# caskcsg/lightretriever

Measured on AMD Instinct MI355X. Metric: docs embedded/sec (llama3.2-1b dims, seq_len=512, bf16) [+ queries/sec@top-100 over 1000000-doc index in `search`], higher is better.
Workload: dtype bf16

## Files before the change

### lightretriever_amd/csrc/lrx_common.h

```cpp
#pragma once
#include <hip/hip_runtime.h>
#include <stdint.h>
#include <stdio.h>
#include <string.h>
#include "../../include/lrx.h"

typedef __attribute__((ext_vector_type(8))) __bf16 bf16x8;
typedef __attribute__((ext_vector_type(4))) __bf16 bf16x4;
typedef __attribute__((ext_vector_type(2))) __bf16 bf16x2;
typedef __attribute__((ext_vector_type(4))) short s16x4;
typedef __attribute__((ext_vector_type(2))) float f32x2;
typedef __attribute__((ext_vector_type(4))) float f32x4;
typedef __attribute__((ext_vector_type(16))) float f32x16;
typedef __attribute__((ext_vector_type(4))) uint32_t u32x4;
typedef __attribute__((ext_vector_type(2))) uint32_t u32x2;

#define LRX_WAVE 64

__device__ __forceinline__ float bf2f(__bf16 v) { return (float)v; }
__device__ __forceinline__ __bf16 f2bf(float v) { return (__bf16)v; }
__device__ __forceinline__ float bfbits2f(uint32_t lo16) { return __uint_as_float(lo16 << 16); }

__device__ __forceinline__ float wave_sum(float v) {
#pragma unroll
// ... 15 lines not shown
}
__device__ __forceinline__ float key2f(uint32_t k) {
  uint32_t u = (k & 0x80000000u) ? (k & 0x7FFFFFFFu) : ~k;
  return __uint_as_float(u);
}
__device__ __forceinline__ unsigned long long sel_pack(uint32_t key, int64_t i) {
  return ((unsigned long long)key << 32) | (unsigned long long)(0xFFFFFFFFu - (uint32_t)i);
}
__device__ __forceinline__ int64_t sel_row(unsigned long long c) { return (int64_t)(0xFFFFFFFFu - (uint32_t)(c & 0xFFFFFFFFull)); }

__host__ __device__ __forceinline__ int64_t lrx_shadow_off(int64_t r, int k, int D) {
  return ((r >> 7) * (int64_t)(D / 64) + (k >> 6)) * 8192 + ((((r >> 4) & 7) * 2 + ((k >> 5) & 1)) * 64 + ((k >> 3) & 3) * 16 + (r & 15)) * 8 + (k & 7);
}

#ifdef LRX_DEV_KNOBS
#include <stdlib.h>
static inline int lrx_dev_knob(const char* name, int dflt) { const char* e = getenv(name); return e ? atoi(e) : dflt; }
#else
static inline int lrx_dev_knob(const char*, int dflt) { return dflt; }
#endif

void lrx_set_error(const char* fmt, ...);
#define LRX_CHECK_ARG(cond, ...)          \
  do {                                    \
    if (!(cond)) {                        \
      lrx_set_error(__VA_ARGS__);         \
      return LRX_ERR_INVALID;             \
    }                                     \
  } while (0)
#define LRX_HIP(call)                                                                     \
  do {                                                                                    \
    hipError_t e_ = (call);                                                               \
    if (e_ != hipSuccess) {                                                               \
      lrx_set_error("%s failed: %s (%s:%d)", #call, hipGetErrorString(e_), __FILE__, __LINE__); \
      return LRX_ERR_HIP;                                                                 \
    }                                                                                     \
  } while (0)
#define LRX_LAUNCH_CHECK() LRX_HIP(hipGetLastError())

static inline int64_t lrx_cdiv(int64_t a, int64_t b) { return (a + b - 1) / b; }

#define LRX_EMIT_MAX_QUERIES 1024
int lrx_gemm_filter_emit_launch(const void* Xb, const void* q16, int64_t n_rows, int nq, int dim, int ss, int64_t n_tiles,
                                const float* thr, unsigned long long* cand, unsigned int* cnt, unsigned int cap, hipStream_t stream);
int lrx_gemm_filter_sample_launch(const void* Xb, const void* q16, int64_t n_rows, int nq, int dim, int ss, int64_t n_tiles, float* scores, float* gmax,
                                  int64_t ld_s, int nblk_ld_s, hipStream_t stream);
int lrx_gemm_max_aggregate_launch(const void* A, const void* B, const void* bias, const int32_t* row_seg, float* out, int64_t ldo, int M, int N,
                                  int K, hipStream_t stream);

int lrx_gemm_nt_fused_ex(const void* A, const void* B, void* C, const void* bias, const void* resid, int32_t M, int32_t N, int32_t K, int32_t epilogue,
                         const float* rscale, float* ss_part, int f16, void* stream);
int lrx_gemm_qkv_rope_slice_ex(const void* A, const void* Wqkv, void* C, const void* bias, const int32_t* positions, const float* cos, const float* sin,
                               int32_t M, int32_t K, int32_t num_q_heads, int32_t num_kv_heads, int32_t head_dim, const float* rscale, int32_t head0,
                               int32_t n_heads, int f16, void* stream);
int lrx_gemm_nt_resid32_ex(const void* A, const void* B, float* x32, void* a16_out, const void* gamma, int32_t M, int32_t N, int32_t K, float* ss_part,
                           int f16, int out_f16, void* stream);
int lrx_attn_varlen_causal_ex(const void* qkv, const int32_t* cu_seqlens, const void* items, size_t items_bytes, int32_t n_seqs, int32_t total_tokens,
                              int32_t max_seqlen, int32_t num_q_heads, int32_t num_kv_heads, int32_t head_dim, void* out, int32_t last_tile_only,
                              int out_f16, void* stream);
int lrx_attn_prefix_suffix_ex(const void* qkv, const void* prefix_kv, int32_t n_seqs, int32_t suffix_len, int32_t prefix_len, int32_t num_q_heads,
                              int32_t num_kv_heads, int32_t head_dim, void* out, int out_f16, void* stream);
int lrx_embed_stream32_ex(const void* table, const int32_t* ids, int32_t n_tokens, int32_t hidden, int32_t vocab, const void* gamma, float* x32, void* a16,
                          float* rscale, float eps, int f16, void* stream);
int lrx_pool_sum_rows(const void* src, int src_kind, const int32_t* ids, int vocab, const int32_t* cu_seqlens, int n_seqs, int hidden_size, float* aux,
                      hipStream_t stream);
int lrx_pool_norm_aux(const void* hidden, const void* final_norm_w, const int32_t* cu_seqlens, int32_t n_seqs, int32_t hidden_size, float eps,
                      int32_t pooling, const float* aux, float* out, int64_t out_row_stride, int32_t out_dim, int32_t normalize, void* shadow_out,
                      int64_t shadow_row0, float* row_bounds, int32_t hidden_f32, void* stream);
int lrx_gather_rows_u32(const void* src, const int32_t* cu_seqlens, int32_t n_seqs, void* dst, hipStream_t stream);
```

### lightretriever_amd/csrc/lrx_gemm.hip

```cpp
#include "lrx_common.h"
#include <float.h>
#include <stdlib.h>

#define GBM 256
#define GBN 256
#define GBK 64
#define HALF_BYTES 16384

enum { EPI_STORE = 0, EPI_RESID = 1, EPI_SWIGLU = 2, EPI_ROPE = 3, EPI_MAXAGG = 4, EPI_EMIT = 5, EPI_RESID32 = 6, EPI_SAMPLE = 7 };
#define EPI_IS_SEARCH(E) ((E) == EPI_EMIT || (E) == EPI_SAMPLE)

struct RopeArgs {
  const int32_t* positions;
  const float* cos;
  const float* sin;
  int rope_cols;
  int head_dim;
  int ldc;
};

__device__ __forceinline__ __bf16 f2h_bits(float v) {
  return __builtin_bit_cast(__bf16, (_Float16)fminf(fmaxf(v, -65504.f), 65504.f));
}
__device__ unsigned int g_qkv_fp16_saturations = 0;
// ... 16 lines not shown
  float* scores;
  float* gmax;
  int64_t ld_s;
  int nblk_ld_s;
};

struct MaxAggArgs {
  const int32_t* row_seg;
  float* out;
  int64_t ldo;
};

struct NormArgs {
  const float* rscale;
  float* ss_part;
  int group_m;
};

__device__ __forceinline__ void atomic_fmax_bits(float* p, float v) {
  const unsigned b = __float_as_uint(v);
  if (!(b & 0x80000000u)) __hip_atomic_fetch_max((int*)p, (int)b, __ATOMIC_RELAXED, __HIP_MEMORY_SCOPE_AGENT);
  else __hip_atomic_fetch_min((unsigned*)p, b, __ATOMIC_RELAXED, __HIP_MEMORY_SCOPE_AGENT);
}

typedef const __attribute__((address_space(1))) void* gptr_t;
typedef __attribute__((address_space(3))) void* lptr_t;

#define G_BAR()                            \
  do {                                     \
    __builtin_amdgcn_sched_barrier(0);     \
    __builtin_amdgcn_s_barrier();          \
    __builtin_amdgcn_sched_barrier(0);     \
  } while (0)
#define G_LSYNC()                                          \
  do {                                                     \
    asm volatile("s_waitcnt lgkmcnt(0)" ::: "memory");     \
    G_BAR();                                               \
  } while (0)



typedef __attribute__((ext_vector_type(8))) _Float16 f16x8;
template <int EPI, bool F16>
__device__ __forceinline__ f32x4 gemm_mfma(bf16x8 x, bf16x8 y, f32x4 c) {
  if constexpr (EPI_IS_SEARCH(EPI) || F16) return __builtin_amdgcn_mfma_f32_16x16x32_f16(__builtin_bit_cast(f16x8, x), __builtin_bit_cast(f16x8, y), c, 0, 0, 0);
  else return __builtin_amdgcn_mfma_f32_16x16x32_bf16(x, y, c, 0, 0, 0);
}

template <int EPI, bool F16 = false, bool OUTH = F16>
__global__ void __launch_bounds__(512, 2)
k_gemm_bf16_nt(const __bf16* __restrict__ A, const __bf16* __restrict__ B, __bf16* C, const __bf16* __restrict__ bias,
               const __bf16* resid, int M, int N, int K, int tiles_m, int tiles_n, RopeArgs rope, MaxAggArgs mx, NormArgs nrm, EmitArgs em) {
  __shared__ __attribute__((aligned(1024))) char smem[8 * HALF_BYTES + (EPI == EPI_EMIT ? 2304 : 0)];
  const int nwg = gridDim.x, bid = blockIdx.x;
  const int xcd = bid & 7, qd = nwg >> 3, rm = nwg & 7;
  const int t_lin = (xcd < rm ? xcd * (qd + 1) : rm * (qd + 1) + (xcd - rm) * qd) + (bid >> 3);
  const int GM = nrm.group_m;
  const int width = GM * tiles_n;
  const int group = t_lin / width, first_m = group * GM;
  const int gsz = min(tiles_m - first_m, GM);
  const int tin = t_lin - group * width;
  const int tm = first_m + tin % gsz, tn = tin / gsz;
  const int tmx = EPI == EPI_SAMPLE ? tm * em.ss : ((EPI == EPI_EMIT && em.ss > 1) ? (tm / (em.ss - 1)) * em.ss + 1 + tm % (em.ss - 1) : tm);
  const int m0 = tmx * GBM, n0 = tn * GBN;

  const int tid = threadIdx.x, lane = tid & 63;
  const int wave = __builtin_amdgcn_readfirstlane(tid >> 6);
  const int wr = wave >> 2, wc = wave & 3;
  if constexpr (EPI == EPI_EMIT) {
    float* xthr = (float*)(smem + 8 * HALF_BYTES);
    unsigned int* xqc = (unsigned int*)(smem + 8 * HALF_BYTES + 1024);
    if (tid < GBN) { xthr[tid] = n0 + tid < N ? em.thr[n0 + tid] : FLT_MAX; xqc[tid] = 0u; }
    if (tid < 8) ((unsigned int*)(smem + 8 * HALF_BYTES + 2048))[tid] = 0u;
  }

  const __bf16 *pA0[2], *pA1[2], *pB0[2], *pB1[2];
#pragma unroll
  for (int i = 0; i < 2; ++i) {
    int s = (wave * 2 + i) * 64 + lane;
    int row = s >> 3, c = (s & 7) ^ ((row >> 1) & 7);
    if (EPI_IS_SEARCH(EPI)) {
      const int64_t lastb = (int64_t)(M - 1) >> 7;
      const int64_t b0 = min((int64_t)(m0 >> 7), lastb), b1 = min((int64_t)(m0 >> 7) + 1, lastb);
      pA0[i] = A + (b0 * (K / 64)) * 8192 + s * 8;
      pA1[i] = A + (b1 * (K / 64)) * 8192 + s * 8;
    } else {
      pA0[i] = A + (int64_t)min(m0 + row, M - 1) * K + c * 8;
      pA1[i] = A + (int64_t)min(m0 + 128 + row, M - 1) * K + c * 8;
    }
    pB0[i] = B + (int64_t)min(n0 + row, N - 1) * K + c * 8;
    pB1[i] = B + (int64_t)min(n0 + 128 + row, N - 1) * K + c * 8;
  }
  char* const dma_dst = smem + wave * 2048;
#define G_KOFF(KT) ((KT) * GBK)
  const int a_ks = EPI_IS_SEARCH(EPI) ? 8192 : GBK;
#define G_ISSUE_(P, SLOT, BUF, KOFF)                                                                                       \
  do {                                                                                                                     \
    __builtin_amdgcn_global_load_lds((gptr_t)(P[0] + (KOFF)), (lptr_t)(dma_dst + (BUF) * 65536 + (SLOT) * HALF_BYTES), 16, 0, 0);        \
    __builtin_amdgcn_global_load_lds((gptr_t)(P[1] + (KOFF)), (lptr_t)(dma_dst + (BUF) * 65536 + (SLOT) * HALF_BYTES + 1024), 16, 0, 0); \
  } while (0)
#define G_ISSUE(P, SLOT, BUF, KT) G_ISSUE_(P, SLOT, BUF, ((SLOT) < 2 ? (int64_t)(KT) * a_ks : (int64_t)G_KOFF(KT)))

  const int fr = lane & 15, fq = lane >> 4;
  const int xs = fr >> 1;
  int laneoff[2];
#pragma unroll
  for (int ks = 0; ks < 2; ++ks) laneoff[ks] = fr * 128 + (((ks * 4 + fq) ^ xs) << 4);
  int laneoffA[2];
#pragma unroll
  for (int ks = 0; ks < 2; ++ks) laneoffA[ks] = EPI_IS_SEARCH(EPI) ? ks * 1024 + lane * 16 : laneoff[ks];
  const int a_off = (wr * 64) * 128, b_off = 2 * HALF_BYTES + (wc * 32) * 128;

  f32x4 acc[2][2][4][2];
#pragma unroll
  for (int h = 0; h < 2; ++h)
#pragma unroll
    for (int hp = 0; hp < 2; ++hp)
#pragma unroll
      for (int mi = 0; mi < 4; ++mi)
#pragma unroll
        for (int ni = 0; ni < 2; ++ni) acc[h][hp][mi][ni] = f32x4{0.f, 0.f, 0.f, 0.f};
  bf16x8 a[4][2], b[2][2];

#define G_LDA(H)                                                                                     \
  _Pragma("unroll") for (int mi = 0; mi < 4; ++mi) _Pragma("unroll") for (int ks = 0; ks < 2; ++ks)  \
      a[mi][ks] = *(const bf16x8*)(sbuf + (H) * HALF_BYTES + a_off + mi * 2048 + laneoffA[ks]);
#define G_LDB(HP)                                                                                    \
  _Pragma("unroll") for (int ni = 0; ni < 2; ++ni) _Pragma("unroll") for (int ks = 0; ks < 2; ++ks)  \
      b[ni][ks] = *(const bf16x8*)(sbuf + (HP) * HALF_BYTES + b_off + ni * 2048 + laneoff[ks]);
#define G_MM(H, HP)                                                                                   \
  do {                                                                                                \
    _Pragma("unroll") for (int ks = 0; ks < 2; ++ks) _Pragma("unroll") for (int mi = 0; mi < 4; ++mi) \
        _Pragma("unroll") for (int ni = 0; ni < 2; ++ni) acc[H][HP][mi][ni] =                        \
            gemm_mfma<EPI, F16>(b[ni][ks], a[mi][ks], acc[H][HP][mi][ni]); \
  } while (0)

  float rsv[2][4];
#pragma unroll
  for (int h = 0; h < 2; ++h)
#pragma unroll
    for (int mi = 0; mi < 4; ++mi)
      rsv[h][mi] = (EPI != EPI_MAXAGG && EPI != EPI_RESID && !EPI_IS_SEARCH(EPI) && nrm.rscale != nullptr) ? nrm.rscale[min(m0 + h * 128 + wr * 64 + mi * 16 + fr, M - 1)] : 1.0f;

  int rposv[2][4];
#pragma unroll
  for (int h = 0; h < 2; ++h)
#pragma unroll
    for (int mi = 0; mi < 4; ++mi) rposv[h][mi] = EPI == EPI_ROPE ? rope.positions[min(m0 + h * 128 + wr * 64 + mi * 16 + fr, M - 1)] : 0;

  const int nk = K / GBK;
  G_ISSUE(pA0, 0, 0, 0); G_ISSUE(pB1, 3, 0, 0); G_ISSUE(pA1, 1, 0, 0); G_ISSUE(pB0, 2, 0, 0);
  if (nk > 1) {
    G_ISSUE(pA0, 0, 1, 1); G_ISSUE(pB0, 2, 1, 1); G_ISSUE(pB1, 3, 1, 1); G_ISSUE(pA1, 1, 1, 1);
    asm volatile("s_waitcnt vmcnt(8)" ::: "memory");
  } else {
    asm volatile("s_waitcnt vmcnt(0)" ::: "memory");
  }

  G_BAR();
  if (wr == 1) G_BAR();

  bf16x8 b2[2][2];
#define G_LDB2(HP)                                                                                   \
  _Pragma("unroll") for (int ni = 0; ni < 2; ++ni) _Pragma("unroll") for (int ks = 0; ks < 2; ++ks)  \
      b2[ni][ks] = *(const bf16x8*)(sbuf + (HP) * HALF_BYTES + b_off + ni * 2048 + laneoff[ks]);
#define G_MM2(H, HP)                                                                                  \
  do {                                                                                                \
    _Pragma("unroll") for (int ks = 0; ks < 2; ++ks) _Pragma("unroll") for (int mi = 0; mi < 4; ++mi) \
        _Pragma("unroll") for (int ni = 0; ni < 2; ++ni) acc[H][HP][mi][ni] =                        \
            gemm_mfma<EPI, F16>(b2[ni][ks], a[mi][ks], acc[H][HP][mi][ni]); \
  } while (0)
  for (int t = 0; t < nk; ++t) {
    const int cur = t & 1;
    const char* sbuf = smem + cur * 65536;
    const bool n1 = t + 1 < nk, n2 = t + 2 < nk;
    G_LDB(0) G_LDB2(1) G_LDA(0)
    if (t >= 1 && n1) G_ISSUE(pA1, 1, cur ^ 1, t + 1);
    if (n1 && n2) asm volatile("s_waitcnt vmcnt(8)" ::: "memory"); else asm volatile("s_waitcnt vmcnt(0)" ::: "memory");
    G_LSYNC();
    __builtin_amdgcn_s_setprio(1);
    G_MM(0, 0); G_MM2(0, 1);
    __builtin_amdgcn_s_setprio(0);
    G_BAR();
    G_LDA(1)
    if (n2) {
      G_ISSUE(pA0, 0, cur, t + 2); G_ISSUE(pB0, 2, cur, t + 2); G_ISSUE(pB1, 3, cur, t + 2);
      asm volatile("s_waitcnt vmcnt(8)" ::: "memory");
    } else {
      asm volatile("s_waitcnt vmcnt(0)" ::: "memory");
    }
    G_LSYNC();
    __builtin_amdgcn_s_setprio(1);
    G_MM2(1, 1); G_MM(1, 0);
    __builtin_amdgcn_s_setprio(0);
    G_BAR();
  }
  if (wr == 0) G_BAR();

  if constexpr (EPI == EPI_SAMPLE) {
    const int64_t gstride = 8 * (int64_t)em.nblk_ld_s;
#pragma unroll
    for (int hp = 0; hp < 2; ++hp) {
      if (hp) __syncthreads();
#pragma unroll
      for (int h = 0; h < 2; ++h)
#pragma unroll
        for (int mi = 0; mi < 4; ++mi) {
          const int row = h * 128 + wr * 64 + mi * 16 + fr;
          const bool mok = (int64_t)m0 + row < M;
#pragma unroll
          for (int ni = 0; ni < 2; ++ni)
#pragma unroll
            for (int r = 0; r < 4; ++r) {
              const int cl = wc * 32 + ni * 16 + fq * 4 + r;
              *(float*)(smem + cl * 1024 + ((((row >> 2) ^ (fq << 2))) << 4) + (row & 3) * 4) = mok ? acc[h][hp][mi][ni][r] : -FLT_MAX;
            }
        }
      __syncthreads();
#pragma unroll 4
      for (int it = 0; it < 16; ++it) {
        const int cl = it * 8 + wave, col = n0 + hp * 128 + cl;
        const f32x4 v = *(const f32x4*)(smem + cl * 1024 + ((lane ^ (((cl >> 2) & 3) << 2)) << 4));
        float mx = fmaxf(fmaxf(v[0], v[1]), fmaxf(v[2], v[3]));
        mx = fmaxf(mx, __int_as_float(__builtin_amdgcn_update_dpp(0, __float_as_int(mx), 0x4E, 0xF, 0xF, true)));
        mx = fmaxf(mx, __int_as_float(__builtin_amdgcn_update_dpp(0, __float_as_int(mx), 0xB1, 0xF, 0xF, true)));
        if (col < N) {
          *(f32x4*)(em.scores + (int64_t)col * em.ld_s + (int64_t)tm * GBM + lane * 4) = v;
          if ((lane & 3) == 0) em.gmax[(int64_t)col * gstride + (int64_t)tm * 16 + (lane >> 2)] = mx;
        }
      }
    }
    return;
  }
  if constexpr (EPI == EPI_EMIT) {
    constexpr int WCAP = 512;
    unsigned long long* wl = (unsigned long long*)(smem + wave * (WCAP * 12 + 64));
    unsigned int* wq = (unsigned int*)(wl + WCAP);
    unsigned int* wn = (unsigned int*)(smem + 8 * HALF_BYTES + 2048) + wave;
    unsigned int* qc = (unsigned int*)(smem + 8 * HALF_BYTES + 1024);
    const float* xthr = (const float*)(smem + 8 * HALF_BYTES);
    f32x4 t16[2][2];
#pragma unroll
    for (int hp = 0; hp < 2; ++hp)
#pragma unroll
      for (int ni = 0; ni < 2; ++ni) t16[hp][ni] = *(const f32x4*)(xthr + hp * 128 + wc * 32 + ni * 16 + fq * 4);
#pragma unroll
    for (int h = 0; h < 2; ++h)
#pragma unroll
      for (int mi = 0; mi < 4; ++mi) {
        const int64_t m = (int64_t)m0 + h * 128 + wr * 64 + mi * 16 + fr;
// ... 54 lines not shown
#pragma unroll
      for (int it = 0; it < 16; ++it) {
        const int m = m0 + p * 128 + it * 8 + wave;
        rv[it] = (m < M && nin) ? *(const f32x4*)(x32 + (int64_t)m * N + nq4) : f32x4{0.f, 0.f, 0.f, 0.f};
      }
      if (p) __syncthreads();
#pragma unroll
      for (int hp = 0; hp < 2; ++hp)
#pragma unroll
        for (int mi = 0; mi < 4; ++mi)
#pragma unroll
          for (int ni = 0; ni < 2; ++ni) {
            const int row = wr * 64 + mi * 16 + fr, chunk = hp * 32 + wc * 8 + ni * 4 + fq;
            *(f32x4*)(smem + row * 1024 + ((chunk ^ ((row & 15) << 2)) << 4)) = acc[p][hp][mi][ni];
          }
      __syncthreads();
#pragma unroll
      for (int it = 0; it < 16; ++it) {
        const int row = it * 8 + wave, m = m0 + p * 128 + row;
        f32x4 v = *(const f32x4*)(smem + row * 1024 + ((lane ^ ((row & 15) << 2)) << 4));
        const bool inb = m < M && nin;
#pragma unroll
        for (int e = 0; e < 4; ++e) v[e] += rv[it][e];
        if (inb) {
          *(f32x4*)(x32 + (int64_t)m * N + nq4) = v;
          if (C != nullptr) {
            bf16x4 a4;
            if constexpr (OUTH) {
              bool sat = false;
#pragma unroll
              for (int e = 0; e < 4; ++e) { const float t = v[e] * gm[e]; sat |= !(fabsf(t) <= 65504.f); a4[e] = f2h_bits(t); }
              if (__any(sat)) { if ((int)(threadIdx.x & 63) == __ffsll((long long)__ballot(1)) - 1) atomicAdd(&g_qkv_fp16_saturations, 1u); }
            } else {
#pragma unroll
              for (int e = 0; e < 4; ++e) a4[e] = f2bf(v[e] * gm[e]);
            }
            *(bf16x4*)(C + (int64_t)m * N + nq4) = a4;
          }
        }
        if (nrm.ss_part != nullptr) {
          float ssq = inb ? (v[0] * v[0] + v[1] * v[1]) + (v[2] * v[2] + v[3] * v[3]) : 0.f;
          ssq += __int_as_float(__builtin_amdgcn_update_dpp(0, __float_as_int(ssq), 0x128, 0xF, 0xF, true));
          ssq += __int_as_float(__builtin_amdgcn_update_dpp(0, __float_as_int(ssq), 0x124, 0xF, 0xF, true));
          ssq += __int_as_float(__builtin_amdgcn_update_dpp(0, __float_as_int(ssq), 0x4E, 0xF, 0xF, true));
          ssq += __int_as_float(__builtin_amdgcn_update_dpp(0, __float_as_int(ssq), 0xB1, 0xF, 0xF, true));
          ssq += __int_as_float(__builtin_amdgcn_update_dpp(0, __float_as_int(ssq), 0x142, 0xA, 0xF, false));
          ssq += __int_as_float(__builtin_amdgcn_update_dpp(0, __float_as_int(ssq), 0x143, 0xC, 0xF, false));
          if (lane == 63 && m < M) nrm.ss_part[(int64_t)tn * M + m] = ssq;
        }
      }
    }
    return;
  }
  constexpr int CW = (EPI == EPI_SWIGLU) ? 128 : 256;
  constexpr int CPR = CW / 8;
  constexpr int NIT = (256 * CPR) / 512;
  bf16x8 rv[EPI == EPI_RESID ? NIT : 1];
  if (EPI == EPI_RESID) {
    const int ldc_ = N, c0_ = n0;
#pragma unroll
    for (int it = 0; it < NIT; ++it) {
      const int q = it * 512 + tid;
      const int m = min(m0 + q / CPR, M - 1), n = min(c0_ + (q % CPR) * 8, ldc_ - 8);
      rv[it] = *(const bf16x8*)(resid + (int64_t)m * N + n);
    }
  }
#pragma unroll
  for (int h = 0; h < 2; ++h)
#pragma unroll
    for (int mi = 0; mi < 4; ++mi) {
      const int row = h * 128 + wr * 64 + mi * 16 + fr;
      const float rs = rsv[h][mi];
#pragma unroll
      for (int hp = 0; hp < 2; ++hp) {
        if (EPI == EPI_SWIGLU) {
          bf16x4 o;
          bool sat = false;
#pragma unroll
          for (int r = 0; r < 4; ++r) {
            const float g = acc[h][hp][mi][0][r] * rs, u = acc[h][hp][mi][1][r] * rs;
            const float sg = __builtin_amdgcn_rcpf(1.0f + __builtin_amdgcn_exp2f(g * -1.4426950408889634f));
            const float t = g * sg * u;
            if constexpr (F16) { sat |= !(fabsf(t) <= 65504.f); o[r] = f2h_bits(t); }
            else o[r] = f2bf(t);
          }
          if constexpr (F16) { if (__any(sat)) { if ((int)(threadIdx.x & 63) == __ffsll((long long)__ballot(1)) - 1) atomicAdd(&g_qkv_fp16_saturations, 1u); } }
          const int col = hp * 64 + wc * 16 + fq * 4;
          *(bf16x4*)(smem + row * (CW * 2) + ((((col >> 3) ^ (row & 15)) << 4) | ((col & 4) << 1))) = o;
        } else if (EPI == EPI_ROPE) {
          const int cb = hp * 128 + wc * 32;
          const bool rot = n0 + cb < rope.rope_cols;
          f32x4 x1 = acc[h][hp][mi][0], x2 = acc[h][hp][mi][1];
#pragma unroll
          for (int r = 0; r < 4; ++r) { x1[r] *= rs; x2[r] *= rs; }
          if (bias != nullptr) {
            const int nb = min(n0 + cb + fq * 4, N - 20);
            const bf16x4 b1 = *(const bf16x4*)(bias + nb), b2 = *(const bf16x4*)(bias + nb + 16);
#pragma unroll
            for (int r = 0; r < 4; ++r) { x1[r] += bf2f(b1[r]); x2[r] += bf2f(b2[r]); }
          }
          if (rot) {
            const int rhalf = rope.head_dim >> 1;
            const int j = (((n0 + cb) % rope.head_dim) >> 5) * 16 + fq * 4;
            const f32x4 cc = *(const f32x4*)(rope.cos + (int64_t)rposv[h][mi] * rhalf + j), sn = *(const f32x4*)(rope.sin + (int64_t)rposv[h][mi] * rhalf + j);
#pragma unroll
            for (int r = 0; r < 4; ++r) {
              const float a = x1[r], b = x2[r];
              x1[r] = a * cc[r] - b * sn[r];
              x2[r] = b * cc[r] + a * sn[r];
            }
          }
          bf16x4 o1, o2;
          bool sat = false;
#pragma unroll
          for (int r = 0; r < 4; ++r) {
            sat |= !(fabsf(x1[r]) <= 65504.f) | !(fabsf(x2[r]) <= 65504.f);
            o1[r] = f2h_bits(x1[r]);
            o2[r] = f2h_bits(x2[r]);
          }
          if (__any(sat)) { if ((int)(threadIdx.x & 63) == __ffsll((long long)__ballot(1)) - 1) atomicAdd(&g_qkv_fp16_saturations, 1u); }
          const int c1 = cb + fq * 4, c2 = c1 + 16;
          *(bf16x4*)(smem + row * (CW * 2) + ((((c1 >> 3) ^ (row & 15)) << 4) | ((c1 & 4) << 1))) = o1;
          *(bf16x4*)(smem + row * (CW * 2) + ((((c2 >> 3) ^ (row & 15)) << 4) | ((c2 & 4) << 1))) = o2;
        } else {
#pragma unroll
          for (int ni = 0; ni < 2; ++ni) {
            const int col = hp * 128 + wc * 32 + ni * 16 + fq * 4;
            f32x4 v = acc[h][hp][mi][ni];
            if (EPI == EPI_STORE) {
#pragma unroll
              for (int r = 0; r < 4; ++r) v[r] *= rs;
            }
            if (EPI == EPI_STORE && bias != nullptr) {
              const int n = min(n0 + col, N - 4);
              bf16x4 bv = *(const bf16x4*)(bias + n);
#pragma unroll
              for (int r = 0; r < 4; ++r) v[r] += bf2f(bv[r]);
            }
            if (EPI == EPI_MAXAGG && bias != nullptr) {
#pragma unroll
              for (int r = 0; r < 4; ++r) v[r] += bf2f(bias[min(n0 + col + r, N - 1)]);
            }
            bf16x4 o;
#pragma unroll
            for (int r = 0; r < 4; ++r) o[r] = f2bf(v[r]);
            *(bf16x4*)(smem + row * (CW * 2) + ((((col >> 3) ^ (row & 15)) << 4) | ((col & 4) << 1))) = o;
          }
        }
      }
    }
  __syncthreads();
  if (EPI == EPI_MAXAGG) {
    const int colq = wave * 32 + (lane & 7) * 4;
    const int choff = colq >> 3, hb = (colq & 4) << 1;
    const float NEG = -__builtin_inff();
    float m4[4] = {NEG, NEG, NEG, NEG};
    int cur = -1;
    auto flush = [&](int seg) {
      if (seg < 0) return;
#pragma unroll
      for (int r = 0; r < 4; ++r)
        if (n0 + colq + r < N && m4[r] != NEG) atomic_fmax_bits(mx.out + (int64_t)seg * mx.ldo + n0 + colq + r, m4[r]);
    };
    for (int step = 0; step < 32; ++step) {
      const int row = step * 8 + (lane >> 3);
      const int m = m0 + row;
      const int seg = m < M ? mx.row_seg[m] : -1;
      if (seg >= 0) {
        if (seg != cur) {
          flush(cur);
          cur = seg;
#pragma unroll
          for (int r = 0; r < 4; ++r) m4[r] = NEG;
        }
        const bf16x4 v = *(const bf16x4*)(smem + row * 512 + (((choff ^ (row & 15)) << 4) | hb));
#pragma unroll
        for (int r = 0; r < 4; ++r) m4[r] = fmaxf(m4[r], bf2f(v[r]));
      }
    }
    int cmax = cur;
#pragma unroll
    for (int o = 32; o >= 1; o >>= 1) cmax = max(cmax, __shfl_xor(cmax, o));
    const bool uniform = __all(cur == cmax || cur == -1);
    if (uniform) {
      if (cur == -1) {
#pragma unroll
        for (int r = 0; r < 4; ++r) m4[r] = NEG;
      }
#pragma unroll
      for (int o = 8; o <= 32; o <<= 1)
#pragma unroll
        for (int r = 0; r < 4; ++r) m4[r] = fmaxf(m4[r], __shfl_xor(m4[r], o));
      if ((lane >> 3) == 0) flush(cmax);
    } else {
      flush(cur);
    }
    return;
  }
  const int ncols = (EPI == EPI_SWIGLU) ? (N >> 1) : N;
  const int ldc = (EPI == EPI_ROPE && rope.ldc > 0) ? rope.ldc : ncols;
  const int c0 = (EPI == EPI_SWIGLU) ? (n0 >> 1) : n0;
  {
#pragma unroll
  for (int it = 0; it < NIT; ++it) {
    const int q = it * 512 + tid;
    const int row = q / CPR, ch = q % CPR;
    const int m = m0 + row, n = c0 + ch * 8;
    const bool inb = m < M && n < ncols;
    if (!(EPI == EPI_RESID && nrm.ss_part != nullptr) && !inb) continue;
    bf16x8 v = *(const bf16x8*)(smem + row * (CW * 2) + ((ch ^ (row & 15)) << 4));
    if (EPI == EPI_RESID) {
#pragma unroll
      for (int e = 0; e < 8; ++e) v[e] = f2bf(bf2f(v[e]) + bf2f(rv[it][e]));
      if (nrm.ss_part != nullptr) {
        float ssq = 0.f;
#pragma unroll
        for (int e = 0; e < 8; ++e) { const float f = bf2f(v[e]); ssq += f * f; }
        if (!inb) ssq = 0.f;
        ssq += __int_as_float(__builtin_amdgcn_update_dpp(0, __float_as_int(ssq), 0x128, 0xF, 0xF, true));
        ssq += __int_as_float(__builtin_amdgcn_update_dpp(0, __float_as_int(ssq), 0x124, 0xF, 0xF, true));
        ssq += __int_as_float(__builtin_amdgcn_update_dpp(0, __float_as_int(ssq), 0x4E, 0xF, 0xF, true));
        ssq += __int_as_float(__builtin_amdgcn_update_dpp(0, __float_as_int(ssq), 0xB1, 0xF, 0xF, true));
        ssq += __shfl_xor(ssq, 16, 64);
        if ((tid & 31) == 0 && m < M) nrm.ss_part[(int64_t)tn * M + m] = ssq;
        if (!inb) continue;
      }
    }
    *(bf16x8*)(C + (int64_t)m * ldc + n) = v;
  }
  }
}

static int gemm_group_m(int epilogue, int K) {
  static const int env = lrx_dev_knob("LRX_GEMM_GM", 0);
  if (env > 0) return env;
  return epilogue == EPI_SWIGLU ? (K >= 4096 ? 8 : 6) : (epilogue == EPI_RESID ? (K <= 4096 ? 6 : 4) : 8);
}

extern "C" int lrx_gemm_bf16_nt(const void* A, const void* B, void* C, const void* bias, const void* resid, int32_t M, int32_t N,
                                int32_t K, int32_t epilogue, void* stream) {
  return lrx_gemm_bf16_nt_fused(A, B, C, bias, resid, M, N, K, epilogue, nullptr, nullptr, stream);
}

extern "C" int lrx_gemm_bf16_nt_fused(const void* A, const void* B, void* C, const void* bias, const void* resid, int32_t M, int32_t N,
                                      int32_t K, int32_t epilogue, const float* rscale, float* ss_part, void* stream) {
  return lrx_gemm_nt_fused_ex(A, B, C, bias, resid, M, N, K, epilogue, rscale, ss_part, 0, stream);
}

int lrx_gemm_nt_fused_ex(const void* A, const void* B, void* C, const void* bias, const void* resid, int32_t M, int32_t N, int32_t K, int32_t epilogue,
                         const float* rscale, float* ss_part, int f16, void* stream) {
  LRX_CHECK_ARG(M >= 0 && N > 0 && K > 0, "gemm: bad shape M=%d N=%d K=%d", M, N, K);
  LRX_CHECK_ARG(!f16 || epilogue == EPI_SWIGLU, "gemm: fp16 operands are served for the SwiGLU epilogue (epilogue %d)", epilogue);
  LRX_CHECK_ARG(K % GBK == 0, "gemm: K=%d must be a multiple of %d", K, GBK);
  LRX_CHECK_ARG(N % 8 == 0, "gemm: N=%d must be a multiple of 8", N);
  LRX_CHECK_ARG(epilogue >= 0 && epilogue <= 2, "gemm: unknown epilogue %d", epilogue);
  LRX_CHECK_ARG(epilogue != EPI_SWIGLU || N % 32 == 0, "gemm: SwiGLU epilogue needs N %% 32 == 0 (N=%d)", N);
  LRX_CHECK_ARG(epilogue != EPI_RESID || resid != nullptr, "gemm: residual epilogue without resid");
  LRX_CHECK_ARG(ss_part == nullptr || epilogue == EPI_RESID, "gemm: ss_part belongs to the residual epilogue");
  LRX_CHECK_ARG(rscale == nullptr || epilogue != EPI_RESID, "gemm: rscale applies to the store / SwiGLU epilogues");
  if (M == 0) return LRX_OK;
  int tiles_m = (int)lrx_cdiv(M, GBM), tiles_n = (int)lrx_cdiv(N, GBN);
  dim3 grid(tiles_m * tiles_n), block(512);
  hipStream_t s = (hipStream_t)stream;
  const __bf16 *a = (const __bf16*)A, *b = (const __bf16*)B, *bi = (const __bf16*)bias, *re = (const __bf16*)resid;
  __bf16* c = (__bf16*)C;
  RopeArgs none = {nullptr, nullptr, nullptr, 0, 64, 0};
  MaxAggArgs nomx = {nullptr, nullptr, 0};
  NormArgs nrm = {rscale, ss_part, gemm_group_m(epilogue, K)};
  switch (epilogue) {
    case EPI_STORE: hipLaunchKernelGGL(k_gemm_bf16_nt<EPI_STORE>, grid, block, 0, s, a, b, c, bi, re, M, N, K, tiles_m, tiles_n, none, nomx, nrm, EmitArgs{nullptr, nullptr, nullptr, 0, 0u, nullptr, nullptr, 0, 0}); break;
    case EPI_RESID: hipLaunchKernelGGL(k_gemm_bf16_nt<EPI_RESID>, grid, block, 0, s, a, b, c, bi, re, M, N, K, tiles_m, tiles_n, none, nomx, nrm, EmitArgs{nullptr, nullptr, nullptr, 0, 0u, nullptr, nullptr, 0, 0}); break;
    default:
      if (f16) hipLaunchKernelGGL((k_gemm_bf16_nt<EPI_SWIGLU, true>), grid, block, 0, s, a, b, c, bi, re, M, N, K, tiles_m, tiles_n, none, nomx, nrm, EmitArgs{nullptr, nullptr, nullptr, 0, 0u, nullptr, nullptr, 0, 0});
      else hipLaunchKernelGGL(k_gemm_bf16_nt<EPI_SWIGLU>, grid, block, 0, s, a, b, c, bi, re, M, N, K, tiles_m, tiles_n, none, nomx, nrm, EmitArgs{nullptr, nullptr, nullptr, 0, 0u, nullptr, nullptr, 0, 0});
      break;
  }
  LRX_LAUNCH_CHECK();
  return LRX_OK;
}

extern "C" int lrx_gemm_qkv_rope(const void* A, const void* Wqkv, void* C, const void* bias, const int32_t* positions, const float* cos,
                                 const float* sin, int32_t M, int32_t K, int32_t num_q_heads, int32_t num_kv_heads, int32_t head_dim,
                                 void* stream) {
  return lrx_gemm_qkv_rope_fused(A, Wqkv, C, bias, positions, cos, sin, M, K, num_q_heads, num_kv_heads, head_dim, nullptr, stream);
}

extern "C" int lrx_gemm_qkv_rope_fused(const void* A, const void* Wqkv, void* C, const void* bias, const int32_t* positions, const float* cos,
                                       const float* sin, int32_t M, int32_t K, int32_t num_q_heads, int32_t num_kv_heads, int32_t head_dim,
                                       const float* rscale, void* stream) {
  return lrx_gemm_qkv_rope_slice(A, Wqkv, C, bias, positions, cos, sin, M, K, num_q_heads, num_kv_heads, head_dim, rscale, 0,
                                 num_q_heads + 2 * num_kv_heads, stream);
}

extern "C" int lrx_gemm_qkv_rope_slice(const void* A, const void* Wqkv, void* C, const void* bias, const int32_t* positions, const float* cos,
                                       const float* sin, int32_t M, int32_t K, int32_t num_q_heads, int32_t num_kv_heads, int32_t head_dim,
                                       const float* rscale, int32_t head0, int32_t n_heads, void* stream) {
  return lrx_gemm_qkv_rope_slice_ex(A, Wqkv, C, bias, positions, cos, sin, M, K, num_q_heads, num_kv_heads, head_dim, rscale, head0, n_heads, 0, stream);
}

int lrx_gemm_qkv_rope_slice_ex(const void* A, const void* Wqkv, void* C, const void* bias, const int32_t* positions, const float* cos, const float* sin,
                               int32_t M, int32_t K, int32_t num_q_heads, int32_t num_kv_heads, int32_t head_dim, const float* rscale, int32_t head0,
                               int32_t n_heads, int f16, void* stream) {
  const int n_all = num_q_heads + 2 * num_kv_heads;
  LRX_CHECK_ARG(M >= 0 && K > 0 && K % GBK == 0, "gemm_qkv_rope: bad shape M=%d K=%d", M, K);
  LRX_CHECK_ARG(head_dim == 64 || head_dim == 128, "gemm_qkv_rope: head_dim=%d unsupported", head_dim);
  LRX_CHECK_ARG(positions && cos && sin, "gemm_qkv_rope: null rope inputs");
  LRX_CHECK_ARG(head0 >= 0 && n_heads > 0 && head0 + n_heads <= n_all, "gemm_qkv_rope: head slice [%d, %d) outside 0..%d", head0, head0 + n_heads, n_all);
  if (M == 0) return LRX_OK;
  const int N = n_heads * head_dim, col0 = head0 * head_dim;
  const int rope_cols = (num_q_heads + num_kv_heads) * head_dim - col0;
  int tiles_m = (int)lrx_cdiv(M, GBM), tiles_n = (int)lrx_cdiv(N, GBN);
  RopeArgs rope = {positions, cos, sin, rope_cols < 0 ? 0 : (rope_cols > N ? N : rope_cols), head_dim, n_all * head_dim};
  if (f16)
    hipLaunchKernelGGL((k_gemm_bf16_nt<EPI_ROPE, true>), dim3(tiles_m * tiles_n), dim3(512), 0, (hipStream_t)stream, (const __bf16*)A,
                       (const __bf16*)Wqkv + (int64_t)col0 * K, (__bf16*)C + col0, bias ? (const __bf16*)bias + col0 : (const __bf16*)nullptr,
                       (const __bf16*)nullptr, M, N, K, tiles_m, tiles_n, rope, MaxAggArgs{nullptr, nullptr, 0}, NormArgs{rscale, nullptr, 8},
                       EmitArgs{nullptr, nullptr, nullptr, 0, 0u, nullptr, nullptr, 0, 0});
  else
  hipLaunchKernelGGL(k_gemm_bf16_nt<EPI_ROPE>, dim3(tiles_m * tiles_n), dim3(512), 0, (hipStream_t)stream, (const __bf16*)A,
                     (const __bf16*)Wqkv + (int64_t)col0 * K, (__bf16*)C + col0, bias ? (const __bf16*)bias + col0 : (const __bf16*)nullptr,
                     (const __bf16*)nullptr, M, N, K, tiles_m, tiles_n, rope, MaxAggArgs{nullptr, nullptr, 0}, NormArgs{rscale, nullptr, 8},
                     EmitArgs{nullptr, nullptr, nullptr, 0, 0u, nullptr, nullptr, 0, 0});
  LRX_LAUNCH_CHECK();
  return LRX_OK;
}

extern "C" int lrx_gemm_bf16_nt_resid32(const void* A, const void* B, float* x32, void* a16_out, const void* gamma, int32_t M, int32_t N, int32_t K,
                                        float* ss_part, void* stream) {
  return lrx_gemm_nt_resid32_ex(A, B, x32, a16_out, gamma, M, N, K, ss_part, 0, 0, stream);
}

int lrx_gemm_nt_resid32_ex(const void* A, const void* B, float* x32, void* a16_out, const void* gamma, int32_t M, int32_t N, int32_t K, float* ss_part,
                           int f16, int out_f16, void* stream) {
  LRX_CHECK_ARG(!f16 || out_f16 || a16_out == nullptr, "gemm_resid32: fp16 operands write an fp16 operand");
  LRX_CHECK_ARG(M >= 0 && N > 0 && K > 0 && K % GBK == 0 && N % 8 == 0, "gemm_resid32: bad shape M=%d N=%d K=%d", M, N, K);
  LRX_CHECK_ARG(x32 != nullptr, "gemm_resid32: null residual stream");
  if (M == 0) return LRX_OK;
  int tiles_m = (int)lrx_cdiv(M, GBM), tiles_n = (int)lrx_cdiv(N, GBN);
  RopeArgs none = {nullptr, nullptr, nullptr, 0, 64, 0};
  if (f16)
    hipLaunchKernelGGL((k_gemm_bf16_nt<EPI_RESID32, true>), dim3(tiles_m * tiles_n), dim3(512), 0, (hipStream_t)stream, (const __bf16*)A, (const __bf16*)B,
                       (__bf16*)a16_out, (const __bf16*)gamma, (const __bf16*)x32, M, N, K, tiles_m, tiles_n, none, MaxAggArgs{nullptr, nullptr, 0},
                       NormArgs{nullptr, ss_part, gemm_group_m(EPI_RESID, K)}, EmitArgs{nullptr, nullptr, nullptr, 0, 0u, nullptr, nullptr, 0, 0});
  else if (out_f16 && a16_out != nullptr)
    hipLaunchKernelGGL((k_gemm_bf16_nt<EPI_RESID32, false, true>), dim3(tiles_m * tiles_n), dim3(512), 0, (hipStream_t)stream, (const __bf16*)A, (const __bf16*)B,
                       (__bf16*)a16_out, (const __bf16*)gamma, (const __bf16*)x32, M, N, K, tiles_m, tiles_n, none, MaxAggArgs{nullptr, nullptr, 0},
                       NormArgs{nullptr, ss_part, gemm_group_m(EPI_RESID, K)}, EmitArgs{nullptr, nullptr, nullptr, 0, 0u, nullptr, nullptr, 0, 0});
  else
  hipLaunchKernelGGL(k_gemm_bf16_nt<EPI_RESID32>, dim3(tiles_m * tiles_n), dim3(512), 0, (hipStream_t)stream, (const __bf16*)A, (const __bf16*)B,
                     (__bf16*)a16_out, (const __bf16*)gamma, (const __bf16*)x32, M, N, K, tiles_m, tiles_n, none, MaxAggArgs{nullptr, nullptr, 0},
                     NormArgs{nullptr, ss_part, gemm_group_m(EPI_RESID, K)}, EmitArgs{nullptr, nullptr, nullptr, 0, 0u, nullptr, nullptr, 0, 0});
  LRX_LAUNCH_CHECK();
  return LRX_OK;
}

#ifndef LRX_MAXAGG_GM
#define LRX_MAXAGG_GM 8
#endif
int lrx_gemm_max_aggregate_launch(const void* A, const void* B, const void* bias, const int32_t* row_seg, float* out, int64_t ldo, int M, int N,
                                  int K, hipStream_t stream) {
  LRX_CHECK_ARG(M >= 0 && N > 0 && K > 0 && K % GBK == 0, "max_aggregate: bad shape M=%d N=%d K=%d (K must be a multiple of %d)", M, N, K, GBK);
  LRX_CHECK_ARG(row_seg && out && ldo >= N, "max_aggregate: bad output spec");
  if (M == 0) return LRX_OK;
  int tiles_m = (int)lrx_cdiv(M, GBM), tiles_n = (int)lrx_cdiv(N, GBN);
  RopeArgs none = {nullptr, nullptr, nullptr, 0, 64, 0};
  MaxAggArgs mx = {row_seg, out, ldo};
  static const int maxagg_gm = lrx_dev_knob("LRX_MAXAGG_GM", 0) > 0 ? lrx_dev_knob("LRX_MAXAGG_GM", 0) : LRX_MAXAGG_GM;
  hipLaunchKernelGGL(k_gemm_bf16_nt<EPI_MAXAGG>, dim3(tiles_m * tiles_n), dim3(512), 0, stream, (const __bf16*)A, (const __bf16*)B, (__bf16*)nullptr,
                     (const __bf16*)bias, (const __bf16*)nullptr, M, N, K, tiles_m, tiles_n, none, mx, NormArgs{nullptr, nullptr, maxagg_gm},
                     EmitArgs{nullptr, nullptr, nullptr, 0, 0u, nullptr, nullptr, 0, 0});
  LRX_LAUNCH_CHECK();
  return LRX_OK;
}

int lrx_gemm_filter_emit_launch(const void* Xb, const void* q16, int64_t n_rows, int nq, int dim, int ss, int64_t n_tiles,
                                const float* thr, unsigned long long* cand, unsigned int* cnt, unsigned int cap, hipStream_t stream) {
  LRX_CHECK_ARG(dim > 0 && dim % GBK == 0 && nq > 0 && nq <= LRX_EMIT_MAX_QUERIES && n_rows < (1ll << 31), "filter_emit: bad shape rows=%lld nq=%d dim=%d",
                (long long)n_rows, nq, dim);
  if (n_tiles <= 0) return LRX_OK;
  const int tiles_n = (nq + GBN - 1) / GBN;
  LRX_CHECK_ARG(n_tiles * tiles_n < (1ll << 31), "filter_emit: %lld tiles", (long long)(n_tiles * tiles_n));
  static const int gm_env = lrx_dev_knob("LRX_EMIT_GM", 0);
  const int gm = gm_env > 0 ? gm_env : (tiles_n == 1 ? 8 : (32 + tiles_n - 1) / tiles_n);
  RopeArgs none = {nullptr, nullptr, nullptr, 0, 64, 0};
  hipLaunchKernelGGL(k_gemm_bf16_nt<EPI_EMIT>, dim3((unsigned)(n_tiles * tiles_n)), dim3(512), 0, stream, (const __bf16*)Xb, (const __bf16*)q16, (__bf16*)nullptr,
                     (const __bf16*)nullptr, (const __bf16*)nullptr, (int)n_rows, nq, dim, (int)n_tiles, tiles_n, none, MaxAggArgs{nullptr, nullptr, 0},
                     NormArgs{nullptr, nullptr, gm}, EmitArgs{thr, cand, cnt, ss, cap, nullptr, nullptr, 0, 0});
  LRX_LAUNCH_CHECK();
  return LRX_OK;
}

int lrx_gemm_filter_sample_launch(const void* Xb, const void* q16, int64_t n_rows, int nq, int dim, int ss, int64_t n_tiles, float* scores, float* gmax,
                                  int64_t ld_s, int nblk_ld_s, hipStream_t stream) {
  LRX_CHECK_ARG(dim > 0 && dim % GBK == 0 && nq > 0 && nq <= LRX_EMIT_MAX_QUERIES && n_rows < (1ll << 31) && ss >= 1 && scores && gmax,
                "filter_sample: bad shape rows=%lld nq=%d dim=%d", (long long)n_rows, nq, dim);
  if (n_tiles <= 0) return LRX_OK;
  const int tiles_n = (nq + GBN - 1) / GBN;
  RopeArgs none = {nullptr, nullptr, nullptr, 0, 64, 0};
  hipLaunchKernelGGL(k_gemm_bf16_nt<EPI_SAMPLE>, dim3((unsigned)(n_tiles * tiles_n)), dim3(512), 0, stream, (const __bf16*)Xb, (const __bf16*)q16, (__bf16*)nullptr,
                     (const __bf16*)nullptr, (const __bf16*)nullptr, (int)n_rows, nq, dim, (int)n_tiles, tiles_n, none, MaxAggArgs{nullptr, nullptr, 0},
                     NormArgs{nullptr, nullptr, tiles_n == 1 ? 8 : (32 + tiles_n - 1) / tiles_n}, EmitArgs{nullptr, nullptr, nullptr, ss, 0u, scores, gmax, ld_s, nblk_ld_s});
  LRX_LAUNCH_CHECK();
  return LRX_OK;
}
```

Baseline: 1328.

## Make QKV-RoPE GEMM persistent and prefetch next tile's first K-slice during epilogue

Turns the QKV+RoPE GEMM into a persistent kernel: the grid is capped to a multiple of 8 CUs and each workgroup loops over tiles. While it runs the RoPE epilogue for the current tile, it issues the LDS DMA loads for the next tile's first K block into the alternate buffer, and the buffer parity is flipped to match. The RoPE epilogue is split into its own path with bias loads hoisted. This is meant to hide launch tail and pipeline-fill latency, at the cost of more complex smem buffer reuse and possible hazards between the epilogue's smem use and the in-flight prefetch.

Result: no change. 1330 (median of 6 runs) (+0.2%).

```diff
diff --git a/lightretriever_amd/csrc/lrx_common.h b/lightretriever_amd/csrc/lrx_common.h
--- a/lightretriever_amd/csrc/lrx_common.h
+++ b/lightretriever_amd/csrc/lrx_common.h
@@ -91,7 +91,7 @@
                          const float* rscale, float* ss_part, int f16, void* stream);
 int lrx_gemm_qkv_rope_slice_ex(const void* A, const void* Wqkv, void* C, const void* bias, const int32_t* positions, const float* cos, const float* sin,
                                int32_t M, int32_t K, int32_t num_q_heads, int32_t num_kv_heads, int32_t head_dim, const float* rscale, int32_t head0,
-                               int32_t n_heads, int f16, void* stream);
+                               int32_t n_heads, int f16, void* stream, int grid = 0);
 int lrx_gemm_nt_resid32_ex(const void* A, const void* B, float* x32, void* a16_out, const void* gamma, int32_t M, int32_t N, int32_t K, float* ss_part,
                            int f16, int out_f16, void* stream);
 int lrx_attn_varlen_causal_ex(const void* qkv, const int32_t* cu_seqlens, const void* items, size_t items_bytes, int32_t n_seqs, int32_t total_tokens,
diff --git a/lightretriever_amd/csrc/lrx_gemm.hip b/lightretriever_amd/csrc/lrx_gemm.hip
--- a/lightretriever_amd/csrc/lrx_gemm.hip
+++ b/lightretriever_amd/csrc/lrx_gemm.hip
@@ -92,7 +92,10 @@
 k_gemm_bf16_nt(const __bf16* __restrict__ A, const __bf16* __restrict__ B, __bf16* C, const __bf16* __restrict__ bias,
                const __bf16* resid, int M, int N, int K, int tiles_m, int tiles_n, RopeArgs rope, MaxAggArgs mx, NormArgs nrm, EmitArgs em) {
   __shared__ __attribute__((aligned(1024))) char smem[8 * HALF_BYTES + (EPI == EPI_EMIT ? 2304 : 0)];
-  const int nwg = gridDim.x, bid = blockIdx.x;
+  constexpr bool PERSIST = EPI == EPI_ROPE;
+  const int nwg = PERSIST ? tiles_m * tiles_n : (int)gridDim.x;
+  int bid = blockIdx.x, pb = 0;
+  do {
   const int xcd = bid & 7, qd = nwg >> 3, rm = nwg & 7;
   const int t_lin = (xcd < rm ? xcd * (qd + 1) : rm * (qd + 1) + (xcd - rm) * qd) + (bid >> 3);
   const int GM = nrm.group_m;
@@ -104,7 +107,9 @@
   const int tmx = EPI == EPI_SAMPLE ? tm * em.ss : ((EPI == EPI_EMIT && em.ss > 1) ? (tm / (em.ss - 1)) * em.ss + 1 + tm % (em.ss - 1) : tm);
   const int m0 = tmx * GBM, n0 = tn * GBN;
 
-  const int tid = threadIdx.x, lane = tid & 63;
+  int tid = threadIdx.x;
+  if constexpr (PERSIST) asm volatile("" : "+v"(tid));
+  const int lane = tid & 63;
   const int wave = __builtin_amdgcn_readfirstlane(tid >> 6);
   const int wr = wave >> 2, wc = wave & 3;
   if constexpr (EPI == EPI_EMIT) {
@@ -189,9 +194,14 @@
     for (int mi = 0; mi < 4; ++mi) rposv[h][mi] = EPI == EPI_ROPE ? rope.positions[min(m0 + h * 128 + wr * 64 + mi * 16 + fr, M - 1)] : 0;
 
   const int nk = K / GBK;
-  G_ISSUE(pA0, 0, 0, 0); G_ISSUE(pB1, 3, 0, 0); G_ISSUE(pA1, 1, 0, 0); G_ISSUE(pB0, 2, 0, 0);
+  if (!PERSIST || pb == 0) {
+    G_ISSUE(pA0, 0, 0, 0); G_ISSUE(pB1, 3, 0, 0); G_ISSUE(pA1, 1, 0, 0); G_ISSUE(pB0, 2, 0, 0);
+  } else {
+    asm volatile("s_waitcnt vmcnt(0)" ::: "memory");
+    __syncthreads();
+  }
   if (nk > 1) {
-    G_ISSUE(pA0, 0, 1, 1); G_ISSUE(pB0, 2, 1, 1); G_ISSUE(pB1, 3, 1, 1); G_ISSUE(pA1, 1, 1, 1);
+    G_ISSUE(pA0, 0, pb ^ 1, 1); G_ISSUE(pB0, 2, pb ^ 1, 1); G_ISSUE(pB1, 3, pb ^ 1, 1); G_ISSUE(pA1, 1, pb ^ 1, 1);
     asm volatile("s_waitcnt vmcnt(8)" ::: "memory");
   } else {
     asm volatile("s_waitcnt vmcnt(0)" ::: "memory");
@@ -211,7 +221,7 @@
             gemm_mfma<EPI, F16>(b2[ni][ks], a[mi][ks], acc[H][HP][mi][ni]); \
   } while (0)
   for (int t = 0; t < nk; ++t) {
-    const int cur = t & 1;
+    const int cur = (t & 1) ^ pb;
     const char* sbuf = smem + cur * 65536;
     const bool n1 = t + 1 < nk, n2 = t + 2 < nk;
     G_LDB(0) G_LDB2(1) G_LDA(0)
@@ -236,6 +246,27 @@
     G_BAR();
   }
   if (wr == 0) G_BAR();
+  auto request_next_k0 = [&]() {
+    const int bidn = bid + (int)gridDim.x;
+    if (bidn < nwg) {
+      const int xcdn = bidn & 7;
+      const int t_linn = (xcdn < rm ? xcdn * (qd + 1) : rm * (qd + 1) + (xcdn - rm) * qd) + (bidn >> 3);
+      const int groupn = t_linn / width, first_mn = groupn * GM;
+      const int gszn = min(tiles_m - first_mn, GM);
+      const int tinn = t_linn - groupn * width;
+      const int m0n = (first_mn + tinn % gszn) * GBM, n0n = (tinn / gszn) * GBN;
+#pragma unroll
+      for (int i = 0; i < 2; ++i) {
+        const int s = (wave * 2 + i) * 64 + lane;
+        const int row = s >> 3, c = (s & 7) ^ ((row >> 1) & 7);
+        char* const dst = dma_dst + 65536 + i * 1024;
+        __builtin_amdgcn_global_load_lds((gptr_t)(A + (int64_t)min(m0n + row, M - 1) * K + c * 8), (lptr_t)(dst + 0 * HALF_BYTES), 16, 0, 0);
+        __builtin_amdgcn_global_load_lds((gptr_t)(B + (int64_t)min(n0n + 128 + row, N - 1) * K + c * 8), (lptr_t)(dst + 3 * HALF_BYTES), 16, 0, 0);
+        __builtin_amdgcn_global_load_lds((gptr_t)(A + (int64_t)min(m0n + 128 + row, M - 1) * K + c * 8), (lptr_t)(dst + 1 * HALF_BYTES), 16, 0, 0);
+        __builtin_amdgcn_global_load_lds((gptr_t)(B + (int64_t)min(n0n + row, N - 1) * K + c * 8), (lptr_t)(dst + 2 * HALF_BYTES), 16, 0, 0);
+      }
+    }
+  };
 
   if constexpr (EPI == EPI_SAMPLE) {
     const int64_t gstride = 8 * (int64_t)em.nblk_ld_s;
@@ -396,6 +427,72 @@
     }
     return;
   }
+  if constexpr (EPI == EPI_ROPE) {
+    const int ldc = rope.ldc > 0 ? rope.ldc : N;
+    const int rhalf = rope.head_dim >> 1;
+    const int jt = (((n0 + wc * 32) % rope.head_dim) >> 5) * 16 + fq * 4;
+    bf16x4 bs1[2], bs2[2];
+#pragma unroll
+    for (int hp = 0; hp < 2; ++hp) {
+      if (bias != nullptr) {
+        const int nb = min(n0 + hp * 128 + wc * 32 + fq * 4, N - 20);
+        bs1[hp] = *(const bf16x4*)(bias + nb);
+        bs2[hp] = *(const bf16x4*)(bias + nb + 16);
+      }
+    }
+    request_next_k0();
+#pragma unroll
+    for (int h = 0; h < 2; ++h) {
+      if (h) __syncthreads();
+#pragma unroll
+      for (int mi = 0; mi < 4; ++mi) {
+        const int row = wr * 64 + mi * 16 + fr;
+        const float rs = rsv[h][mi];
+#pragma unroll
+        for (int hp = 0; hp < 2; ++hp) {
+          const int cb = hp * 128 + wc * 32;
+          const bool rot = n0 + cb < rope.rope_cols;
+          f32x4 x1 = acc[h][hp][mi][0], x2 = acc[h][hp][mi][1];
+#pragma unroll
+          for (int r = 0; r < 4; ++r) { x1[r] *= rs; x2[r] *= rs; }
+          if (bias != nullptr) {
+#pragma unroll
+            for (int r = 0; r < 4; ++r) { x1[r] += bf2f(bs1[hp][r]); x2[r] += bf2f(bs2[hp][r]); }
+          }
+          if (rot) {
+            const f32x4 cc = *(const f32x4*)(rope.cos + (int64_t)rposv[h][mi] * rhalf + jt), sn = *(const f32x4*)(rope.sin + (int64_t)rposv[h][mi] * rhalf + jt);
+#pragma unroll
+            for (int r = 0; r < 4; ++r) {
+              const float a = x1[r], b = x2[r];
+              x1[r] = a * cc[r] - b * sn[r];
+              x2[r] = b * cc[r] + a * sn[r];
+            }
+          }
+          bf16x4 o1, o2;
+          bool sat = false;
+#pragma unroll
+          for (int r = 0; r < 4; ++r) {
+            sat |= !(fabsf(x1[r]) <= 65504.f) | !(fabsf(x2[r]) <= 65504.f);
+            o1[r] = f2h_bits(x1[r]);
+            o2[r] = f2h_bits(x2[r]);
+          }
+          if (__any(sat)) { if ((int)(threadIdx.x & 63) == __ffsll((long long)__ballot(1)) - 1) atomicAdd(&g_qkv_fp16_saturations, 1u); }
+          const int c1 = cb + fq * 4, c2 = c1 + 16;
+          *(bf16x4*)(smem + row * 512 + ((((c1 >> 3) ^ (row & 15)) << 4) | ((c1 & 4) << 1))) = o1;
+          *(bf16x4*)(smem + row * 512 + ((((c2 >> 3) ^ (row & 15)) << 4) | ((c2 & 4) << 1))) = o2;
+        }
+      }
+      __syncthreads();
+#pragma unroll
+      for (int it = 0; it < 8; ++it) {
+        const int q = it * 512 + tid;
+        const int row = q >> 5, ch = q & 31;
+        const int m = m0 + h * 128 + row, n = n0 + ch * 8;
+        if (m < M && n < N) *(bf16x8*)(C + (int64_t)m * ldc + n) = *(const bf16x8*)(smem + row * 512 + ((ch ^ (row & 15)) << 4));
+      }
+    }
+    continue;
+  }
   constexpr int CW = (EPI == EPI_SWIGLU) ? 128 : 256;
   constexpr int CPR = CW / 8;
   constexpr int NIT = (256 * CPR) / 512;
@@ -431,41 +528,6 @@
           if constexpr (F16) { if (__any(sat)) { if ((int)(threadIdx.x & 63) == __ffsll((long long)__ballot(1)) - 1) atomicAdd(&g_qkv_fp16_saturations, 1u); } }
           const int col = hp * 64 + wc * 16 + fq * 4;
           *(bf16x4*)(smem + row * (CW * 2) + ((((col >> 3) ^ (row & 15)) << 4) | ((col & 4) << 1))) = o;
-        } else if (EPI == EPI_ROPE) {
-          const int cb = hp * 128 + wc * 32;
-          const bool rot = n0 + cb < rope.rope_cols;
-          f32x4 x1 = acc[h][hp][mi][0], x2 = acc[h][hp][mi][1];
-#pragma unroll
-          for (int r = 0; r < 4; ++r) { x1[r] *= rs; x2[r] *= rs; }
-          if (bias != nullptr) {
-            const int nb = min(n0 + cb + fq * 4, N - 20);
-            const bf16x4 b1 = *(const bf16x4*)(bias + nb), b2 = *(const bf16x4*)(bias + nb + 16);
-#pragma unroll
-            for (int r = 0; r < 4; ++r) { x1[r] += bf2f(b1[r]); x2[r] += bf2f(b2[r]); }
-          }
-          if (rot) {
-            const int rhalf = rope.head_dim >> 1;
-            const int j = (((n0 + cb) % rope.head_dim) >> 5) * 16 + fq * 4;
-            const f32x4 cc = *(const f32x4*)(rope.cos + (int64_t)rposv[h][mi] * rhalf + j), sn = *(const f32x4*)(rope.sin + (int64_t)rposv[h][mi] * rhalf + j);
-#pragma unroll
-            for (int r = 0; r < 4; ++r) {
-              const float a = x1[r], b = x2[r];
-              x1[r] = a * cc[r] - b * sn[r];
-              x2[r] = b * cc[r] + a * sn[r];
-            }
-          }
-          bf16x4 o1, o2;
-          bool sat = false;
-#pragma unroll
-          for (int r = 0; r < 4; ++r) {
-            sat |= !(fabsf(x1[r]) <= 65504.f) | !(fabsf(x2[r]) <= 65504.f);
-            o1[r] = f2h_bits(x1[r]);
-            o2[r] = f2h_bits(x2[r]);
-          }
-          if (__any(sat)) { if ((int)(threadIdx.x & 63) == __ffsll((long long)__ballot(1)) - 1) atomicAdd(&g_qkv_fp16_saturations, 1u); }
-          const int c1 = cb + fq * 4, c2 = c1 + 16;
-          *(bf16x4*)(smem + row * (CW * 2) + ((((c1 >> 3) ^ (row & 15)) << 4) | ((c1 & 4) << 1))) = o1;
-          *(bf16x4*)(smem + row * (CW * 2) + ((((c2 >> 3) ^ (row & 15)) << 4) | ((c2 & 4) << 1))) = o2;
         } else {
 #pragma unroll
           for (int ni = 0; ni < 2; ++ni) {
@@ -542,7 +604,7 @@
     return;
   }
   const int ncols = (EPI == EPI_SWIGLU) ? (N >> 1) : N;
-  const int ldc = (EPI == EPI_ROPE && rope.ldc > 0) ? rope.ldc : ncols;
+  const int ldc = ncols;
   const int c0 = (EPI == EPI_SWIGLU) ? (n0 >> 1) : n0;
   {
 #pragma unroll
@@ -573,6 +635,15 @@
     *(bf16x8*)(C + (int64_t)m * ldc + n) = v;
   }
   }
+  } while (PERSIST && (pb = 1, bid += (int)gridDim.x) < nwg);
+}
+
+static unsigned gemm_persistent_grid(int tiles, int grid) {
+  if (grid > 0) return (unsigned)min(grid, tiles);
+  int dev = 0, n_cu = 0;
+  if (hipGetDevice(&dev) != hipSuccess || hipDeviceGetAttribute(&n_cu, hipDeviceAttributeMultiprocessorCount, dev) != hipSuccess) n_cu = 0;
+  const int slots = (n_cu / 8) * 8;
+  return (unsigned)(slots > 0 && slots < tiles ? slots : tiles);
 }
 
 static int gemm_group_m(int epilogue, int K) {
@@ -644,7 +715,7 @@
 
 int lrx_gemm_qkv_rope_slice_ex(const void* A, const void* Wqkv, void* C, const void* bias, const int32_t* positions, const float* cos, const float* sin,
                                int32_t M, int32_t K, int32_t num_q_heads, int32_t num_kv_heads, int32_t head_dim, const float* rscale, int32_t head0,
-                               int32_t n_heads, int f16, void* stream) {
+                               int32_t n_heads, int f16, void* stream, int grid) {
   const int n_all = num_q_heads + 2 * num_kv_heads;
   LRX_CHECK_ARG(M >= 0 && K > 0 && K % GBK == 0, "gemm_qkv_rope: bad shape M=%d K=%d", M, K);
   LRX_CHECK_ARG(head_dim == 64 || head_dim == 128, "gemm_qkv_rope: head_dim=%d unsupported", head_dim);
@@ -655,13 +726,14 @@
   const int rope_cols = (num_q_heads + num_kv_heads) * head_dim - col0;
   int tiles_m = (int)lrx_cdiv(M, GBM), tiles_n = (int)lrx_cdiv(N, GBN);
   RopeArgs rope = {positions, cos, sin, rope_cols < 0 ? 0 : (rope_cols > N ? N : rope_cols), head_dim, n_all * head_dim};
+  const dim3 wgs(gemm_persistent_grid(tiles_m * tiles_n, grid));
   if (f16)
-    hipLaunchKernelGGL((k_gemm_bf16_nt<EPI_ROPE, true>), dim3(tiles_m * tiles_n), dim3(512), 0, (hipStream_t)stream, (const __bf16*)A,
+    hipLaunchKernelGGL((k_gemm_bf16_nt<EPI_ROPE, true>), wgs, dim3(512), 0, (hipStream_t)stream, (const __bf16*)A,
                        (const __bf16*)Wqkv + (int64_t)col0 * K, (__bf16*)C + col0, bias ? (const __bf16*)bias + col0 : (const __bf16*)nullptr,
                        (const __bf16*)nullptr, M, N, K, tiles_m, tiles_n, rope, MaxAggArgs{nullptr, nullptr, 0}, NormArgs{rscale, nullptr, 8},
                        EmitArgs{nullptr, nullptr, nullptr, 0, 0u, nullptr, nullptr, 0, 0});
   else
-  hipLaunchKernelGGL(k_gemm_bf16_nt<EPI_ROPE>, dim3(tiles_m * tiles_n), dim3(512), 0, (hipStream_t)stream, (const __bf16*)A,
+  hipLaunchKernelGGL(k_gemm_bf16_nt<EPI_ROPE>, wgs, dim3(512), 0, (hipStream_t)stream, (const __bf16*)A,
                      (const __bf16*)Wqkv + (int64_t)col0 * K, (__bf16*)C + col0, bias ? (const __bf16*)bias + col0 : (const __bf16*)nullptr,
                      (const __bf16*)nullptr, M, N, K, tiles_m, tiles_n, rope, MaxAggArgs{nullptr, nullptr, 0}, NormArgs{rscale, nullptr, 8},
                      EmitArgs{nullptr, nullptr, nullptr, 0, 0u, nullptr, nullptr, 0, 0});
@@ -747,3 +819,10 @@
   LRX_LAUNCH_CHECK();
   return LRX_OK;
 }
+
+extern "C" int lrx_dev_gemm_qkv_rope_grid(const void* A, const void* Wqkv, void* C, const void* bias, const int32_t* positions, const float* cos,
+                                          const float* sin, int32_t M, int32_t K, int32_t num_q_heads, int32_t num_kv_heads, int32_t head_dim,
+                                          const float* rscale, int32_t head0, int32_t n_heads, int32_t f16, int32_t grid, void* stream) {
+  return lrx_gemm_qkv_rope_slice_ex(A, Wqkv, C, bias, positions, cos, sin, M, K, num_q_heads, num_kv_heads, head_dim, rscale, head0, n_heads, f16,
+                                    stream, grid);
+}
```
